# filthyrake/telescope_cam_detection

Hardware: AMD Instinct MI355X
Metric: frames_per_sec (higher is better)
Workload: dtype f16x3; 1 GPU; RT-DETR-R50 640x640 bs=8/GPU, uint8 BGR frames resident in HBM -> [8,300,6] detections in HBM; synthetic seeded weights; global_batch=8, parallelism=camera-shard x1, streams_per_gpu=1, batches_in_flight_per_gpu=1, hip_graph=True

## Files before the change

telescope_cam_detection_amd/_capi.py:

```python
from __future__ import annotations

import ctypes as C
import os
from typing import Optional

import numpy as np

from . import build as _build
from .arch import Arch

RTD_OK, RTD_E_INVALID, RTD_E_OOM, RTD_E_HIP, RTD_E_WEIGHTS, RTD_E_STATE = range(6)
PREC_BF16, PREC_FP32, PREC_F16X3 = 0, 1, 2
DT_BF16, DT_F32, DT_F16X2 = 0, 1, 4
SPLIT_GROUP = 32


def precision_code(name) -> int:
    if isinstance(name, int):
        return name
    s = str(name).lower()
    if s in ("f16x3", "fp16x3", "pair"):
        return PREC_F16X3
    if s in ("fp32", "f32", "float32"):
        return PREC_FP32
# ... 62 lines not shown

class RtdEnhanceParams(C.Structure):
    _fields_ = [("struct_size", C.c_int32), ("clip_limit", C.c_float), ("tiles_x", C.c_int32), ("tiles_y", C.c_int32),
                ("bilateral_d", C.c_int32), ("sigma_color", C.c_float), ("sigma_space", C.c_float)]


class RtdEsrganConfig(C.Structure):
    _fields_ = [("struct_size", C.c_int32), ("device", C.c_int32), ("precision", C.c_int32), ("num_feat", C.c_int32),
                ("num_grow_ch", C.c_int32), ("num_block", C.c_int32), ("tile", C.c_int32), ("tile_pad", C.c_int32)]


DET_DTYPE = np.dtype([("class_id", "<i4"), ("score", "<f4"), ("x1", "<f4"), ("y1", "<f4"), ("x2", "<f4"), ("y2", "<f4")])

_lib: Optional[C.CDLL] = None

EXPORTS = [
    "rtd_version", "rtd_create", "rtd_load_weights", "rtd_infer", "rtd_infer_raw", "rtd_infer_async", "rtd_collect", "rtd_prepare",
    "rtd_result_block", "rtd_sync", "rtd_stream", "rtd_wait_stream", "rtd_signal_stream", "rtd_get_stats", "rtd_arena_bytes", "rtd_destroy",
    "rtd_last_error", "rtd_crop_resize_batch", "rtd_self_check", "rtd_preprocess",
    "rtd_motion_create", "rtd_motion_check", "rtd_motion_reset", "rtd_motion_wait_stream", "rtd_motion_last_error", "rtd_motion_destroy",
    "rtd_mog2_create", "rtd_mog2_configure", "rtd_mog2_apply", "rtd_mog2_wait_stream", "rtd_mog2_last_error", "rtd_mog2_destroy",
    "rtd_jpeg_create", "rtd_jpeg_encode", "rtd_jpeg_wait_stream", "rtd_jpeg_last_error", "rtd_jpeg_destroy",
    "rtd_overlay_create", "rtd_overlay_draw", "rtd_overlay_wait_stream", "rtd_overlay_last_error", "rtd_overlay_destroy",
    "rtd_enhance_create", "rtd_enhance_layout", "rtd_enhance_crops", "rtd_enhance_last_error", "rtd_enhance_destroy",
    "rtd_esrgan_create", "rtd_esrgan_layout", "rtd_esrgan_upscale", "rtd_esrgan_arena_bytes", "rtd_esrgan_last_error", "rtd_esrgan_destroy",
]
TEST_EXPORTS = [
    "rtd_debug_tensor", "rtd_debug_force_topk", "rtd_profile", "rtd_debug_option", "rtd_op_conv", "rtd_op_conv_dual", "rtd_op_conv_next",
    "rtd_op_layernorm", "rtd_op_attention", "rtd_op_msdeform", "rtd_op_topk", "rtd_op_resize", "rtd_op_pool", "rtd_bench_conv", "rtd_bench_conv_pair",
    "rtd_bench_mfma_rate", "rtd_debug_motion_state", "rtd_debug_mog2_model", "rtd_debug_mog2_fg_bits",
    "rtd_debug_jpeg_coefficients", "rtd_debug_overlay_tiles", "rtd_debug_enhance_stage",
    "rtd_op_conv_view", "rtd_bench_conv_act", "rtd_debug_esrgan_tensor",
    "rtd_op_msdeform_view", "rtd_op_select_score", "rtd_op_gather_ln", "rtd_op_split_convert", "rtd_op_set_rows", "rtd_op_rowmax",
    "rtd_op_gather_rows", "rtd_op_boxes", "rtd_op_add", "rtd_op_postprocess",
]


def lib() -> C.CDLL:
    global _lib
    if _lib is not None:
        return _lib
    path = _build.LIB_PATH
    override = os.environ.get("RTD_LIB_PATH")
    if override:
        if not os.path.exists(override):
            raise RuntimeError(f"RTD_LIB_PATH={override} does not exist")
        path = override
    elif _build.needs_build():
        try:
            path = _build.build(verbose=False)
        except Exception as e:
            if not os.path.exists(path):
                raise RuntimeError(f"libmi355rtdetr.so is missing and cannot be built: {e}") from e
    try:
        import torch
    except Exception:
        pass
    L = C.CDLL(path)
    vp, i32, f32, i64 = C.c_void_p, C.c_int32, C.c_float, C.c_int64
    L.rtd_version.restype = C.c_char_p
    L.rtd_last_error.restype = C.c_char_p
    L.rtd_last_error.argtypes = [vp]
    L.rtd_create.argtypes = [C.POINTER(RtdConfig), C.POINTER(vp)]
    L.rtd_load_weights.argtypes = [vp, vp, C.c_size_t]
    L.rtd_infer.argtypes = [vp, i32, C.POINTER(vp), C.POINTER(i32), i32, f32, i32, vp, C.POINTER(i32)]
    L.rtd_infer_raw.argtypes = [vp, i32, C.POINTER(vp), C.POINTER(i32), i32, vp, vp, vp]
    L.rtd_infer_async.argtypes = [vp, i32, C.POINTER(vp), C.POINTER(i32), i32]
# ... 76 lines not shown
    if hasattr(L, "rtd_enhance_create"):
        L.rtd_enhance_create.argtypes = [i32, C.POINTER(RtdEnhanceParams), C.POINTER(vp)]
        L.rtd_enhance_layout.argtypes = [i32, C.POINTER(i32), C.POINTER(i64)]
        L.rtd_enhance_crops.argtypes = [vp, i32, C.POINTER(vp), C.POINTER(i32), C.POINTER(i32), vp, i64, vp]
        L.rtd_enhance_last_error.argtypes = [vp]
        L.rtd_enhance_last_error.restype = C.c_char_p
        L.rtd_enhance_destroy.argtypes = [vp]
        L.rtd_enhance_destroy.restype = None
        L.rtd_debug_enhance_stage.argtypes = [vp, i32, i32, vp, C.c_size_t]
    if hasattr(L, "rtd_esrgan_create"):
        L.rtd_esrgan_create.argtypes = [C.POINTER(RtdEsrganConfig), vp, C.c_size_t, C.POINTER(vp)]
        L.rtd_esrgan_layout.argtypes = [i32, C.POINTER(i32), C.POINTER(i64)]
        L.rtd_esrgan_upscale.argtypes = [vp, i32, C.POINTER(vp), C.POINTER(i32), C.POINTER(i32), vp, i64, vp]
        L.rtd_esrgan_arena_bytes.argtypes = [vp]
        L.rtd_esrgan_arena_bytes.restype = i64
        L.rtd_esrgan_last_error.argtypes = [vp]
        L.rtd_esrgan_last_error.restype = C.c_char_p
        L.rtd_esrgan_destroy.argtypes = [vp]
        L.rtd_esrgan_destroy.restype = None
        L.rtd_debug_esrgan_tensor.argtypes = [vp, C.c_char_p, vp, i64, C.POINTER(i64)]
        L.rtd_op_conv_view.argtypes = [i32, vp, i32, vp, vp, vp, i32, vp, i32] + [i32] * 10
        L.rtd_bench_conv_act.argtypes = [i32] * 13 + [C.POINTER(f32)]
    if hasattr(L, "rtd_op_select_score"):
        L.rtd_op_msdeform_view.argtypes = [i32, vp, i32, i32, vp, vp, vp] + [i32] * 6 + [C.POINTER(i32), f32]
        L.rtd_op_select_score.argtypes = [vp, i32, vp, vp, vp, vp, vp, i32, i32, i32, i32]
        L.rtd_op_gather_ln.argtypes = [vp, i32, i32, vp, i32, i32, vp, vp, vp, i32]
        L.rtd_op_split_convert.argtypes = [i32, vp, vp, i64, i32, i64, i64]
        L.rtd_op_set_rows.argtypes = [i32, vp, i32, i32, vp, i32, i32, vp, i32]
        L.rtd_op_rowmax.argtypes = [vp, i32, i32, i32, vp]
        L.rtd_op_gather_rows.argtypes = [i32, vp, i32, i32, vp, i32, i32, i32, vp, i32]
        L.rtd_op_boxes.argtypes = [vp, i32, i32, vp, vp, vp, i32, vp]
        L.rtd_op_add.argtypes = [i32, i32, i32, vp, vp, vp, i32, i32, i32, i32]
        L.rtd_op_postprocess.argtypes = [vp, vp, vp, i32, i32, i32, i32, i32, vp]
    _lib = L
    return L


def debug_option(name: str, value: int) -> None:
    rc = lib().rtd_debug_option(name.encode(), int(value))
    if rc != RTD_OK:
        raise ValueError(f"unknown debug option {name!r}")


class RtdError(RuntimeError):
    def __init__(self, code: int, msg: str):
        super().__init__(f"rtd error {code}: {msg}")
        self.code = code


def _stats_of(handle) -> dict:
    st = RtdStats()
    if not handle or lib().rtd_get_stats(handle, C.byref(st)) != RTD_OK:
        return {}
    return {k: (float(getattr(st, k)) if k == "max_abs_filter" else int(getattr(st, k))) for k, _ in RtdStats._fields_ if k not in ("struct_size", "reserved")}


def _raise_msg(code: int, what: str, msg: bytes, suffix: str = ""):
    msg = (msg or b"").decode(errors="replace") + suffix
    if code == RTD_E_OOM:
        import torch
        raise torch.cuda.OutOfMemoryError(f"HIP out of memory in {what}: {msg}")
    raise RtdError(code, msg)


def _raise(code: int, handle=None) -> None:
    assert handle is None
# ... 271 lines not shown
```

telescope_cam_detection_amd/csrc/common.h:

```cpp
#pragma once
#include <hip/hip_runtime.h>
#include <stdint.h>
#include <string.h>

#include <stdexcept>
#include <string>
#include <tuple>
#include <type_traits>
#include <utility>
#include <vector>

#include "error.h"

namespace rtd {

enum DType : int { BF16 = 0, F32 = 1, U8 = 2, I32 = 3, F16X2 = 4 };
constexpr int SPLIT_GROUP = 32;
enum Act : int { ACT_NONE = 0, ACT_RELU = 1, ACT_SILU = 2, ACT_GELU = 3, ACT_LRELU = 4  };
enum ResMode : int { RES_NONE = 0, RES_PRE = 1, RES_POST = 2 };

inline size_t dtype_size(int dt) { return dt == BF16 ? 2 : (dt == U8 ? 1 : 4); }

typedef __bf16 bf16;
typedef __bf16 bf16x8 __attribute__((ext_vector_type(8)));
// ... 138 lines not shown
                      float eps, hipStream_t s);
void launch_add(const Tensor& a, const Tensor& b, const Tensor& y, hipStream_t s);
void launch_axpby(float alpha, const Tensor& a, const Tensor& b, const Tensor& y, hipStream_t s);
void launch_maxpool3x3s2(const Tensor& x, const Tensor& y, hipStream_t s);
void launch_upsample2x(const Tensor& x, const Tensor& y, hipStream_t s);
void launch_avgpool2(const Tensor& x, const Tensor& y, hipStream_t s);
void launch_attention(const Tensor& qk, const Tensor& v, const Tensor& o, int heads, hipStream_t s);
void launch_set_rows(const Tensor& y, const int32_t* rows, int nrows, int rows_per_image, const float* vec,
                     hipStream_t s);
void launch_rowmax(const Tensor& x, float* out, hipStream_t s);
void launch_topk(const float* keys, int B, int N, int K, int32_t* idx, float* vals, hipStream_t s);
void launch_gather_rows(const Tensor& src, const int32_t* idx, int rows_per_image, const Tensor& dst, hipStream_t s);
void launch_ref_init(const Tensor& boxdelta, const float* anchors, const int32_t* idx, int S, float* ref_unact8,
                     float* ref8, hipStream_t s);
void launch_msdeform(const Tensor& value, int value_coff, const Tensor& offaw, const float* ref8, const Tensor& out,
                     int heads, int hd, int n_levels, int n_points, const int32_t* level_hw_start, float offset_scale,
                     hipStream_t s);
void launch_box_refine(const Tensor& delta, float* ref8, hipStream_t s);
void launch_postprocess_scores(const Tensor& logits, float* scores, hipStream_t s);
bool postprocess_fused_supported(const Tensor& logits, int B, int Q);
void launch_postprocess_fused(const Tensor& logits, const float* ref8, const float* scale_wh, int B, int Q, float* block6, hipStream_t s);
void launch_postprocess_gather(const float* topv, const int32_t* topi, const float* ref8, const float* scale_wh,
                               int B, int Q, int C, float* block6, hipStream_t s);
constexpr int RTD_MAX_BATCH = 64;
struct FrameArgs {
  const uint8_t* ptr[RTD_MAX_BATCH];
  float scale_wh[2 * RTD_MAX_BATCH];
  int n;
};
void launch_preprocess_identity(const FrameArgs& fa, int H, int W, const Tensor& y, float* scale_wh_dev, hipStream_t s);
void launch_set_scale(const FrameArgs& fa, float* scale_wh_dev, hipStream_t s);
void launch_set_frame_table(const FrameArgs& fa, const uint8_t** table_dev, float* scale_wh_dev, hipStream_t s);
void launch_stem0_u8(const uint8_t* const* table_dev, int n, int H, int W, const void* w, int Kpad, const float* bias, const Tensor& y, int act,
                     hipStream_t s);
struct ResizeCoef {
  const int32_t* hb;
  const int32_t* hk;
  const int32_t* vb;
  const int32_t* vk;
  int hks, vks;
};
void launch_resize_pil(const uint8_t* src, int sh, int sw, uint8_t* tmp, const Tensor& y, int image, const ResizeCoef& coef,
                       hipStream_t s);
void launch_u8_hwc_to_chw_f32(const uint8_t* src, int H, int W, float* out, hipStream_t s);
void launch_resize_pil_u8(const uint8_t* src, int sh, int sw, uint8_t* tmp, uint8_t* dst, int dh, int dw, const ResizeCoef& c, hipStream_t s);
struct DecLin {
  const float* w;
  const float* b;
  int ldw, N, K;
};
struct DecLN {
  const float* g;
  const float* b;
};

struct DecArgs {
  int mode;
  int attn_split;
  int split;
  int B, Q, D, heads, S, n_levels, n_points, ffn, C;
  float offset_scale;
  const float* q_in;
  const float* kfrag_in;
  const float* vfrag_in;
  const float* hs_in;
  float* hs_out;
  const float* qpos_in;
// ... 105 lines not shown
```

telescope_cam_detection_amd/csrc/engine.hip:

```cpp
#include "engine_internal.h"

using namespace rtd;
using namespace rtd_eng;

namespace rtd {
__thread GraphBuild* t_graph_build = nullptr;
__thread long long t_launches = 0;
}

void launch_force_idx(int32_t* dst, const int32_t* src, const int32_t* flag, int n, hipStream_t s);

namespace rtd_eng {
PlanOpts g_opts;
}

namespace rtd_eng {

void parse_blob(rtd_engine* e) {
  const char* b = e->blob.data();
  const size_t n = e->blob.size();
  RTD_CHECK(n >= 12 && memcmp(b, "RTDW", 4) == 0, RTD_E_WEIGHTS, "weight blob: bad magic");
  uint32_t ver, count;
  memcpy(&ver, b + 4, 4);
  memcpy(&count, b + 8, 4);
// ... 471 lines not shown
    int si, bi, stride, oh, ow, cin, cout;
    bool last, fold_sc;
    Tensor res, sc_in, out;
  };
  void stem(Flow& F);
  void backbone_stage(Flow& F, int si, int cin);
  void shortcut(Flow& F, Block& b);
  void bottleneck_body(Flow& F, const StageBufs& sb, const Block& b);
  void basic_body(Flow& F, const StageBufs& sb, const Block& b);
  Tensor aifi_fused(const Tensor& t0), aifi_by_op(const Tensor& t0);
  Tensor csp(const std::string& pfx, const Tensor& cat, const std::string& oname, const Tensor* up_src = nullptr);
  Tensor encoder(Flow& F);
  bool dec_fused() const { return e->opts.dec_fused && c.d_model == 256 && c.dec_heads == 8 && c.dec_ffn <= 1024 && c.num_classes <= 512 && c.n_levels == 3 && c.n_points == 4; }
  Queries select_queries(Flow& F, const Tensor& mem);
  Decoded decoder(Flow& F, const Tensor& mem, const Queries& q);
  Tensor decoder_fused(Flow& F, const Queries& q, const Tensor& vall, float* ref8, float* ref_unact8);
  Tensor decoder_by_op(const Queries& q, const Tensor& vall, const Tensor& ref8t, float* ref_unact8);
  void post_process(const Decoded& d);
};

void Builder::stem(Flow& F) {
  const int H = c.input_h, W = c.input_w;
  Tensor x = act(SP ? F32 : P, n, H, W, 8, "input");
  plan->input = x;
  const int eh = c.embedding_size / 2;
  const int h = down2(H), w = down2(W);
  Tensor s0 = act(P, n, h, w, eh);
  plan->stem_fused = SP && e->opts.stem_fused_split && eh == 32;
  if (plan->stem_fused) {
    const uint8_t** table = (const uint8_t**)alloc((size_t)c.max_batch * sizeof(void*));
    plan->frame_table = table;
    if (!dry) {
      DevWeight w0 = get_weight(e, {{"backbone.stem.0", 9 * 8}}, P, eh);
      const void* wp = w0.w; const float* bp = w0.bias; const int kp = w0.Kpad; const int n = this->n;
      push("backbone.stem.0", "conv_igemm", 2.0 * n * h * w * eh * 27.0, (double)n * H * W * 3 + tbytes(s0),
           [table, n, H, W, wp, kp, bp, s0](hipStream_t st) { launch_stem0_u8(table, n, H, W, wp, kp, bp, s0, ACT_RELU, st); });
    }
  } else {
    conv("backbone.stem.0", x, s0, {.k = 3, .stride = 2, .pad = 1, .act = ACT_RELU, .real_cin = 3});
  }
  Tensor s1 = act(P, n, h, w, eh);
  conv("backbone.stem.1", s0, s1, {.k = 3, .pad = 1, .act = ACT_RELU});
  const Tensor s2v = mk(nullptr, P, n, h, w, c.embedding_size);
  const int ph = down2(h), pw = down2(w);
  const ConvSpec stem2{.k = 3, .pad = 1, .act = ACT_RELU};
  const long long pool_tiles = (long long)n * ((w + 31) / 32) * ((h + 7) / 8);
  const bool fuse = SP && e->opts.stem_pool_fuse && conv_pool_supported(probe(s1, s2v, stem2), probe_shape(mk(nullptr, P, n, ph, pw, c.embedding_size), 1)) &&
                    pool_tiles * 8192 < (1ll << 31);
  F.h = ph; F.w = pw;
  if (fuse) {
    F.cur = act(P, n, ph, pw, c.embedding_size, "stem");
    ConvArgs a;
    a.x = s1; a.y = s2v;
    a.KH = a.KW = 3; a.stride = 1; a.pad = 1; a.act = ACT_RELU; a.opts = &e->conv_opts;
    const DevWeight w2 = get_weight(e, {{"backbone.stem.2", 9 * s1.c}}, P, c.embedding_size, dry);
    a.w = w2.w; a.bias = w2.bias; a.Kpad = w2.Kpad; a.Npad = w2.Npad;
    void* side = alloc(conv_pool_side_bytes(a));
    const Tensor curv = F.cur;
    push("backbone.stem.2+pool", "conv_igemm", 2.0 * s2v.pixels() * s2v.c * 9.0 * s1.c, tbytes(s1) + tbytes(curv),
         [a, curv, side](hipStream_t st) { launch_conv_pool(a, curv, side, st); });
  } else {
    Tensor s2 = act(P, n, h, w, c.embedding_size);
    conv("backbone.stem.2", s1, s2, stem2);
    F.cur = act(P, n, ph, pw, c.embedding_size, "stem");
    const Tensor curv = F.cur;
    push("backbone.pool", "maxpool", 9.0 * curv.pixels() * curv.c, tbytes(s2) + tbytes(curv),
         [s2, curv](hipStream_t s) { launch_maxpool3x3s2(s2, curv, s); });
  }
}
// ... 1064 lines not shown
```

telescope_cam_detection_amd/csrc/engine_internal.h:

```cpp
#pragma once
#include <math.h>
#include <string.h>

#include <chrono>
#include <functional>
#include <map>
#include <memory>
#include <mutex>
#include <string>
#include <vector>

#include "../../include/rtdetr_mi355_test.h"
#include "backend.h"

namespace rtd_eng {
using namespace rtd;

struct PlanOpts {
  int sc_fold = 1;
  int c1_fuse = 1;
  int attn_split = 3;
  int up_fold = 1;
  int arena_reuse = 1;
  int stem_fused_split = 1;
  int aifi_pair = 1;
  int post_fused = 1;
  int dead_out = 1;
  int avg_fuse = 1;
  int stem_pool_fuse = 1;
  int sel_fused = 1;
  int dec_fused = 1;
  int side_stream = 7;
};

struct HostTensor {
  const float* data = nullptr;
  std::vector<int64_t> shape;
  int64_t numel() const {
    int64_t n = 1;
    for (auto d : shape) n *= d;
    return n;
  }
};

struct DevWeight {
  void* w = nullptr;
  float* bias = nullptr;
  int N = 0, K = 0, Kpad = 0, Npad = 0, dt = F32;
};

struct Op {
  std::string name;
  const char* kernel;
  double flops, bytes;
  std::function<void(hipStream_t)> run;
  bool debug_only = false;
  int lane = 0, kind = 0;
// ... 106 lines not shown
```

telescope_cam_detection_amd/csrc/ops.hip:

```cpp
#include <float.h>

#include <algorithm>

#include "common.h"

namespace rtd {

template <typename T> __device__ __forceinline__ float ldf(const T* p) { return (float)(*p); }
template <typename T> __device__ __forceinline__ void stf(T* p, float v) { *p = (T)v; }

__device__ __forceinline__ float wave_sum(float v) { return wave_sum64(v); }

static inline unsigned blocks_for(int64_t n, int per_block) { return (unsigned)((n + per_block - 1) / per_block); }

template <typename... KArgs, typename... Args>
static void launch_1d(void (*kernel)(KArgs...), int64_t total, hipStream_t s, Args&&... args) {
  rtd_launch(kernel, dim3(blocks_for(total, 256)), dim3(256), 0, s, std::forward<Args>(args)...);
  HIP_CHECK(hipGetLastError());
}

template <typename T> struct TypeTag { typedef T type; };
template <typename Tag> using type_of = typename Tag::type;
template <typename F>
static void with_dtype(int dt, F&& f) {
// ... 1084 lines not shown
    o[2] = (T)((float)v[0] / 255.0f);
#pragma unroll
    for (int q = 3; q < 8; ++q) o[q] = (T)0.f;
  }
}
void launch_resize_pil(const uint8_t* src, int sh, int sw, uint8_t* tmp, const Tensor& y, int image, const ResizeCoef& c,
                       hipStream_t s) {
  const int dh = y.h, dw = y.w;
  RTD_CHECK(y.c == 8 && y.ld == 8 && image < y.n, 1, "resize: output must be [n,H,W,8]");
  launch_1d(k_resize_h, (int64_t)sh * dw, s, src, sh, sw, tmp, dw, c);
  char* yp = (char*)y.p + (size_t)image * y.bstride * dtype_size(y.dt);
  with_dtype(y.dt, [&](auto t) { typedef type_of<decltype(t)> T; launch_1d(k_resize_v<T>, (int64_t)dh * dw, s, tmp, sh, dw, (T*)yp, dh, c); });
}
void launch_resize_pil_u8(const uint8_t* src, int sh, int sw, uint8_t* tmp, uint8_t* dst, int dh, int dw, const ResizeCoef& c, hipStream_t s) {
  launch_1d(k_resize_h, (int64_t)sh * dw, s, src, sh, sw, tmp, dw, c);
  launch_1d(k_resize_v<uint8_t>, (int64_t)dh * dw, s, tmp, sh, dw, dst, dh, c);
}

__global__ void k_u8_hwc_to_chw_f32(const uint8_t* __restrict__ src, int H, int W, float* __restrict__ out) {
  const int64_t i = (int64_t)blockIdx.x * blockDim.x + threadIdx.x;
  const int64_t hw = (int64_t)H * W;
  if (i >= hw) return;
  const uint8_t* px = src + i * 3;
  out[i] = (float)px[2] / 255.0f;
  out[hw + i] = (float)px[1] / 255.0f;
  out[2 * hw + i] = (float)px[0] / 255.0f;
}
void launch_u8_hwc_to_chw_f32(const uint8_t* src, int H, int W, float* out, hipStream_t s) {
  launch_1d(k_u8_hwc_to_chw_f32, (int64_t)H * W, s, src, H, W, out);
}

typedef float f32x16_s __attribute__((ext_vector_type(16)));
typedef float f32x4_s __attribute__((ext_vector_type(4)));
__global__ __launch_bounds__(256) void stem0_u8_kernel(const uint8_t* const* __restrict__ table, int H, int W, const sp16* __restrict__ wq, int Kpad,
                                                        const float* __restrict__ bias, sp16* __restrict__ y, long long y_bstride, long long ldy,
                                                        int OH, int OW, int tiles_x, int tiles_y, int act) {
  constexpr bool SPLIT = true;
  typedef sp16 E;
  typedef E Ex8 __attribute__((ext_vector_type(8)));
  typedef E Ex4 __attribute__((ext_vector_type(4)));
  constexpr int TH = 8, TW = 32, PR = 2 * TH + 1, PC = 2 * TW + 1, ROWE = 200;
  constexpr int NDW = (PC * 3 + 3 + 3) / 4;
  constexpr int ROWO = (SPLIT ? 128 : 64) + 16;
  __shared__ __attribute__((aligned(16))) E patch[PR * ROWE];
  __shared__ __attribute__((aligned(16))) E patch_lo[SPLIT ? PR * ROWE : 8];
  __shared__ __attribute__((aligned(16))) char stage[4][32 * ROWO];
  const int tid = threadIdx.x, lane = tid & 63, wv = tid >> 6, h = lane >> 5;
  int t = blockIdx.x;
  const int tx = t % tiles_x; t /= tiles_x;
  const int ty = t % tiles_y;
  const int b = t / tiles_y;
  const int x0 = tx * TW, y0 = ty * TH;
  const uint8_t* __restrict__ f = table[b];
  const long long fbytes = (long long)H * W * 3;
  const bool aligned4 = (((uintptr_t)f) & 3) == 0;
  for (int e = tid; e < PR * NDW; e += 256) {
    const int r = e / NDW, d = e - r * NDW;
    const int iy = 2 * y0 - 1 + r;
    const long long g0 = ((long long)iy * W + (2 * x0 - 1)) * 3;
    const long long a0 = (g0 & ~3ll) + 4ll * d;
    unsigned dw = 0;
    const bool row_ok = (unsigned)iy < (unsigned)H;
    if (row_ok) {
      if (aligned4 && a0 >= 0 && a0 + 4 <= fbytes) dw = *(const unsigned*)(f + a0);
      else {
#pragma unroll
        for (int q = 0; q < 4; ++q)
          if (a0 + q >= 0 && a0 + q < fbytes) dw |= (unsigned)f[a0 + q] << (8 * q);
      }
    }
#pragma unroll
    for (int q = 0; q < 4; ++q) {
      const int el = (int)(a0 + q - g0);
      if (el < 0 || el >= PC * 3) continue;
      const int ix = 2 * x0 - 1 + el / 3;
      const float v = (row_ok && (unsigned)ix < (unsigned)W) ? (float)((dw >> (8 * q)) & 0xffu) : 0.f;
      const float vn = v / 255.0f;
      const E hi = (E)vn;
      patch[r * ROWE + el] = hi;
      if (SPLIT) patch_lo[r * ROWE + el] = (E)(vn - (float)hi);
    }
  }
  for (int e = tid; e < PR * (ROWE - PC * 3); e += 256) {
    const int r = e / (ROWE - PC * 3), i = e - r * (ROWE - PC * 3);
    patch[r * ROWE + PC * 3 + i] = (E)0.f;
    if (SPLIT) patch_lo[r * ROWE + PC * 3 + i] = (E)0.f;
  }
  Ex8 wf[2], wfl[2];
  int doff[2][4];
#pragma unroll
  for (int s = 0; s < 2; ++s) {
#pragma unroll
    for (int j = 0; j < 8; ++j) {
      const int k = 16 * s + 8 * h + j;
      const int kh = k / 10, e = k - kh * 10;
      const int kw = e / 3, cb = e - kw * 3;
      const int kr = (kh * 3 + kw) * 8 + (2 - cb);
      const bool real = k < 30 && e < 9;
      if (SPLIT) {
        const size_t pos = (size_t)(lane & 31) * Kpad + ((kr >> 5) << 6) + (kr & 31);
        wf[s][j] = real ? wq[pos] : (E)0.f;
        wfl[s][j] = real ? wq[pos + 32] : (E)0.f;
      } else {
        wf[s][j] = real ? wq[(size_t)(lane & 31) * Kpad + kr] : (E)0.f;
      }
    }
#pragma unroll
    for (int j = 0; j < 4; ++j) {
      const int k = 16 * s + 8 * h + 2 * j;
      const int kh = k / 10, e = k - kh * 10;
      doff[s][j] = k < 30 ? kh * ROWE + e : 0;
    }
  }
  __syncthreads();
#pragma unroll 1
  for (int rr = 0; rr < 2; ++rr) {
    const int r = wv * 2 + rr;
    const int eoff = (2 * r) * ROWE + (2 * (lane & 31)) * 3;
    const E* base = patch + eoff;
    f32x16_s acc;
#pragma unroll
    for (int e = 0; e < 16; ++e) acc[e] = 0.f;
#pragma unroll
    for (int s = 0; s < 2; ++s) {
      typedef unsigned u4_s __attribute__((ext_vector_type(4)));
      unsigned xd[4];
#pragma unroll
      for (int j = 0; j < 4; ++j) xd[j] = *(const unsigned*)(base + doff[s][j]);
      const u4_s xv = {xd[0], xd[1], xd[2], xd[3]};
      if constexpr (SPLIT) acc = mfma_pair32(wf[s], __builtin_bit_cast(Ex8, xv), acc);
      else acc = __builtin_amdgcn_mfma_f32_32x32x16_bf16(wf[s], __builtin_bit_cast(Ex8, xv), acc, 0, 0, 0);
      if constexpr (SPLIT) {
        unsigned xl[4];
#pragma unroll
        for (int j = 0; j < 4; ++j) xl[j] = *(const unsigned*)(patch_lo + eoff + doff[s][j]);
        const u4_s xlv = {xl[0], xl[1], xl[2], xl[3]};
        acc = mfma_pair32(wf[s], __builtin_bit_cast(Ex8, xlv), acc);
        acc = mfma_pair32(wfl[s], __builtin_bit_cast(Ex8, xv), acc);
      }
    }
    const int oy = y0 + r;
    char* sw_ = stage[wv];
#pragma unroll
    for (int q = 0; q < 4; ++q) {
      const f32x4_s bv = *(const f32x4_s*)(bias + 8 * q + 4 * h);
      Ex4 o, ol;
#pragma unroll
      for (int e = 0; e < 4; ++e) {
        float v = acc[4 * q + e] + bv[e];
        if (act == ACT_RELU) v = fmaxf(v, 0.f);
        else if (act == ACT_SILU) v = v / (1.f + __expf(-v));
        if constexpr (SPLIT) { sp16 hh, ll; split2(v, hh, ll); o[e] = hh; ol[e] = ll; }
        else o[e] = (E)v;
      }
      *(Ex4*)(sw_ + (lane & 31) * ROWO + (8 * q + 4 * h) * 2) = o;
      if (SPLIT) *(Ex4*)(sw_ + (lane & 31) * ROWO + 64 + (8 * q + 4 * h) * 2) = ol;
    }
    __builtin_amdgcn_wave_barrier();
    if (oy < OH) {
      constexpr int CPP = SPLIT ? 8 : 4;
      E* yrow = y + (SPLIT ? 2 : 1) * ((long long)b * y_bstride + ((long long)oy * OW + x0) * ldy);
#pragma unroll
      for (int i2 = 0; i2 < CPP / 2; ++i2) {
        const int idx = i2 * 64 + lane;
        const int p = idx / CPP, ch = idx % CPP;
        if (x0 + p < OW) *(Ex8*)(yrow + (SPLIT ? 2 : 1) * (long long)p * ldy + ch * 8) = *(const Ex8*)(sw_ + p * ROWO + ch * 16);
      }
    }
    __builtin_amdgcn_wave_barrier();
  }
}
void launch_stem0_u8(const uint8_t* const* table_dev, int n, int H, int W, const void* w, int Kpad, const float* bias, const Tensor& y, int act,
                     hipStream_t s) {
  const int OH = (H + 2 - 3) / 2 + 1, OW = (W + 2 - 3) / 2 + 1;
  RTD_CHECK(y.dt == F16X2 && y.c == 32 && y.h == OH && y.w == OW && y.n >= n && y.ld % SPLIT_GROUP == 0 &&
                (act == ACT_RELU || act == ACT_NONE || act == ACT_SILU), 1, "stem0_u8: output must be F16X2 [n, H/2, W/2, 32]");
  const int tiles_x = (OW + 31) / 32, tiles_y = (OH + 7) / 8;
  rtd_launch(stem0_u8_kernel, dim3((unsigned)(n * tiles_x * tiles_y)), dim3(256), 0, s, table_dev, H, W, (const sp16*)w, Kpad, bias, (sp16*)y.p,
                     (long long)y.bstride, (long long)y.ld, OH, OW, tiles_x, tiles_y, act);
  HIP_CHECK(hipGetLastError());
}

struct CropNorm { float mean[3], inv_std[3]; };
__global__ void k_crop_resize(const CropBatch cb, int n, int S, CropNorm nm, float* __restrict__ out) {
  const int64_t i = (int64_t)blockIdx.x * blockDim.x + threadIdx.x;
  const int64_t per = (int64_t)S * S;
  if (i >= per * n) return;
  const int c = (int)(i / per);
  const int p = (int)(i - (int64_t)c * per);
  const int oy = p / S, ox = p - oy * S;
  const int cw = cb.x2[c] - cb.x1[c], chh = cb.y2[c] - cb.y1[c];
  const float sx = (float)cw / (float)S, sy = (float)chh / (float)S;
  const float fx = fmaxf(sx * ((float)ox + 0.5f) - 0.5f, 0.f), fy = fmaxf(sy * ((float)oy + 0.5f) - 0.5f, 0.f);
  const int x0 = min((int)fx, cw - 1), y0 = min((int)fy, chh - 1);
  const int x1 = min(x0 + 1, cw - 1), y1 = min(y0 + 1, chh - 1);
  const float lx1 = fx - (float)x0, ly1 = fy - (float)y0, lx0 = 1.f - lx1, ly0 = 1.f - ly1;
  const uint8_t* f = cb.frame[c];
  const int64_t fw = cb.fw[c];
  const uint8_t* p00 = f + ((int64_t)(cb.y1[c] + y0) * fw + cb.x1[c] + x0) * 3;
  const uint8_t* p01 = f + ((int64_t)(cb.y1[c] + y0) * fw + cb.x1[c] + x1) * 3;
  const uint8_t* p10 = f + ((int64_t)(cb.y1[c] + y1) * fw + cb.x1[c] + x0) * 3;
  const uint8_t* p11 = f + ((int64_t)(cb.y1[c] + y1) * fw + cb.x1[c] + x1) * 3;
#pragma unroll
  for (int ch = 0; ch < 3; ++ch) {
    const int sc = 2 - ch;
    const float v = ly0 * (lx0 * (float)p00[sc] + lx1 * (float)p01[sc]) + ly1 * (lx0 * (float)p10[sc] + lx1 * (float)p11[sc]);
    out[((int64_t)c * 3 + ch) * per + p] = (v / 255.0f - nm.mean[ch]) * nm.inv_std[ch];
  }
}
void launch_crop_resize(const CropBatch& cb, int n, int out_size, const float mean[3], const float stdv[3], float* out, hipStream_t s) {
  RTD_CHECK(n >= 1 && n <= 64 && out_size >= 1 && out_size <= 4096, 1, "crop batch: 1..64 crops per launch");
  for (int i = 0; i < n; ++i) {
// ... 11 lines not shown
```

telescope_cam_detection_amd/csrc/testapi.hip:

```cpp
#include "engine_internal.h"

using namespace rtd;
using namespace rtd_eng;

struct OpScratch {
  std::vector<void*> bufs;
  template <typename T> T* get(size_t count) {
    void* p = nullptr;
    HIP_CHECK(hipMalloc(&p, count ? count * sizeof(T) : 16));
    bufs.push_back(p);
    return (T*)p;
  }
  template <typename T> T* upload(const T* host, size_t count) {
    T* d = get<T>(count);
    HIP_CHECK(hipMemcpy(d, host, count * sizeof(T), hipMemcpyHostToDevice));
    return d;
  }
  ~OpScratch() { for (void* p : bufs) (void)hipFree(p); }
};
static bool rows_fit_int(int a, int b) { return a >= 1 && b >= 1 && (int64_t)a * b <= 0x7fffffff; }
static Tensor rows_view(const void* p, int dt, int n, int rows, int c, int64_t ld) {
  Tensor t = mk(p, dt, n, rows, 1, c);
  t.ld = ld; t.bstride = (int64_t)rows * ld;
  return t;
// ... 151 lines not shown
  sp16x8 a[4], b[4];
  for (int i = 0; i < 4; ++i)
    for (int j = 0; j < 8; ++j) {
      const unsigned h = seed[(lane * 8 + j + i * 512) & 4095];
      a[i][j] = __builtin_bit_cast(sp16, (unsigned short)h);
      b[i][j] = __builtin_bit_cast(sp16, (unsigned short)(h >> 16));
    }
  f32x4 acc[16];
  for (int i = 0; i < 16; ++i) acc[i] = f32x4{0.f, 0.f, 0.f, 0.f};
  const long long c0 = __builtin_amdgcn_s_memtime(), r0 = __builtin_amdgcn_s_memrealtime();
  for (int it = 0; it < iters; ++it) {
#pragma unroll
    for (int i = 0; i < 16; ++i) asm volatile("v_mfma_f32_16x16x32_f16 %0, %1, %2, %0" : "+v"(acc[i]) : "v"(a[i & 3]), "v"(b[(i >> 2) & 3]));
  }
  asm volatile("s_nop 15\n\ts_nop 15\n\ts_nop 15" ::: "memory");
  __builtin_amdgcn_s_waitcnt(0);
  const long long c1 = __builtin_amdgcn_s_memtime(), r1 = __builtin_amdgcn_s_memrealtime();
  float s = 0.f;
  for (int i = 0; i < 16; ++i) s += acc[i][0] + acc[i][3];
  if (s == 123.456f) sink[0] = s;
  if (lane == 0) { const int w = blockIdx.x * 4 + (tid >> 6); out[2 * w] = c1 - c0; out[2 * w + 1] = r1 - r0; }
}
static int g_bench_rewarm = 0;
int rtd_debug_option(const char* name, int value) {
  if (!name) return RTD_E_INVALID;
  if (strcmp(name, "reset") == 0) {
    g_opts = PlanOpts();
    g_profile_twice = 0; g_bench_rewarm = 0;
    conv_opts_template() = ConvOpts();
    return RTD_OK;
  }
  const struct { const char* n; int* p; } plan_opts[] = {
      {"dec_fused", &g_opts.dec_fused}, {"side_stream", &g_opts.side_stream}, {"sel_fused", &g_opts.sel_fused},
      {"stem_fused_split", &g_opts.stem_fused_split}, {"stem_pool_fuse", &g_opts.stem_pool_fuse}, {"avg_fuse", &g_opts.avg_fuse}, {"dead_out", &g_opts.dead_out}, {"post_fused", &g_opts.post_fused}, {"aifi_pair", &g_opts.aifi_pair}, {"sc_fold", &g_opts.sc_fold}, {"arena_reuse", &g_opts.arena_reuse},
      {"up_fold", &g_opts.up_fold}, {"attn_split", &g_opts.attn_split}, {"c1_fuse", &g_opts.c1_fuse},
      {"profile_twice", &g_profile_twice}, {"bench_rewarm", &g_bench_rewarm},
  };
  for (const auto& t : plan_opts)
    if (strcmp(name, t.n) == 0) { *t.p = value; return RTD_OK; }
  if (conv_set_option(name, value)) return RTD_OK;
  return RTD_E_INVALID;
}

struct DevFilter {
  float* wpad = nullptr; void* w = nullptr; float* bias = nullptr;
  int Kpad = 0, Npad = 0;
  void release() { if (w != wpad) (void)hipFree(w); (void)hipFree(wpad); (void)hipFree(bias); }
};
static DevFilter dev_filter(int dtype, const void* w_f32, const float* bias, int N, int K) {
  DevFilter f;
  f.Npad = conv_npad(N);
  f.Kpad = dtype == F16X2 ? conv_kpad_split(K) : conv_kpad(K);
  const int kcols = dtype == F16X2 ? f.Kpad / 2 : f.Kpad;
  HIP_CHECK(hipMalloc((void**)&f.wpad, (size_t)f.Npad * kcols * 4));
  HIP_CHECK(hipMemset(f.wpad, 0, (size_t)f.Npad * kcols * 4));
  HIP_CHECK(hipMemcpy2D(f.wpad, (size_t)kcols * 4, w_f32, (size_t)K * 4, (size_t)K * 4, N, hipMemcpyDeviceToDevice));
  HIP_CHECK(hipMalloc((void**)&f.bias, (size_t)f.Npad * 4));
  HIP_CHECK(hipMemset(f.bias, 0, (size_t)f.Npad * 4));
  HIP_CHECK(hipMemcpy(f.bias, bias, (size_t)N * 4, hipMemcpyDeviceToDevice));
  f.w = f.wpad;
  if (dtype == BF16 || dtype == F16X2) HIP_CHECK(hipMalloc(&f.w, (size_t)f.Npad * f.Kpad * 2));
  if (dtype == BF16) launch_f32_to(f.wpad, f.w, BF16, (int64_t)f.Npad * f.Kpad, nullptr);
  else if (dtype == F16X2) launch_f32_to_split(f.wpad, kcols, f.w, kcols, f.Npad, kcols, nullptr);
  return f;
}

static int op_conv_impl(int dtype, const void* x, const void* x2, int C2, const void* w_ohwi_f32, const float* bias, const void* res, void* y,
// ... 218 lines not shown
    const int cus = prop.multiProcessorCount;
    std::vector<unsigned> hs(4096, 0u);
    if (random_operands)
      for (int i = 0; i < 4096; ++i) {
        unsigned h = (unsigned)i * 2654435761u + 12345u; h ^= h >> 15; h *= 2246822519u; h ^= h >> 13;
        const unsigned lo = (h & 0x8000u) | ((10u + ((h >> 20) & 7u)) << 10) | (h & 0x3ffu);
        unsigned h2 = h * 2654435761u; h2 ^= h2 >> 16;
        const unsigned hi = (h2 & 0x8000u) | ((10u + ((h2 >> 20) & 7u)) << 10) | (h2 & 0x3ffu);
        hs[i] = lo | (hi << 16);
      }
    Scratch sc;
    HIP_CHECK(hipMalloc((void**)&sc.seed, 4096 * 4)); HIP_CHECK(hipMalloc((void**)&sc.stamps, (size_t)cus * 4 * 2 * 8)); HIP_CHECK(hipMalloc((void**)&sc.sink, 16));
    HIP_CHECK(hipMemcpy(sc.seed, hs.data(), 4096 * 4, hipMemcpyHostToDevice));
    const int iters = ms_target * 9400;
    HIP_CHECK(hipEventCreate(&sc.e0)); HIP_CHECK(hipEventCreate(&sc.e1));
    float ms = 0.f;
    for (int rep = 0; rep < 3; ++rep) {
      HIP_CHECK(hipEventRecord(sc.e0, nullptr));
      rtd_launch(k_mfma_rate, dim3(cus), dim3(256), 0, nullptr, sc.seed, iters, sc.stamps, sc.sink);
      HIP_CHECK(hipEventRecord(sc.e1, nullptr));
      HIP_CHECK(hipEventSynchronize(sc.e1));
      HIP_CHECK(hipEventElapsedTime(&ms, sc.e0, sc.e1));
    }
    std::vector<long long> h((size_t)cus * 4 * 2);
    HIP_CHECK(hipMemcpy(h.data(), sc.stamps, h.size() * 8, hipMemcpyDeviceToHost));
    double cyc = 0, rt = 0;
    for (int w = 0; w < cus * 4; ++w) { cyc += (double)h[2 * w]; rt += (double)h[2 * w + 1]; }
    out[0] = (float)((double)iters * 16.0 * cus * 4.0 * 16384.0 / (ms * 1e-3) / 1e12);
    out[1] = (float)(cyc / (rt * 10.0));
    out[2] = ms;
  });
}

int rtd_op_layernorm(int dtype, const void* x, const void* res, const float* g, const float* b, void* y, int rows, int dim, int out_f32) {
  return op_guard([&] {
    Tensor tx = mk(x, dtype, 1, rows, 1, dim), ty = mk(y, out_f32 ? F32 : dtype, 1, rows, 1, dim), tr = mk(res, dtype, 1, rows, 1, dim);
    launch_layernorm(tx, res ? &tr : nullptr, g, b, ty, 1e-5f, nullptr);
  });
}

int rtd_op_attention(int dtype, const void* qk, const void* v, void* o, int B, int L, int heads, int hd) {
  return op_guard([&] {
    const int D = heads * hd;
    launch_attention(mk(qk, dtype, B, L, 1, 2 * D), mk(v, dtype, B, L, 1, D), mk(o, dtype, B, L, 1, D), heads, nullptr);
  });
}

int rtd_op_msdeform(int dtype, const void* value, const float* offaw, const float* ref, float* out, int B, int Q, int heads, int hd,
                    int n_levels, int n_points, const int32_t* level_hw, int value_ld, float offset_scale) {
  return op_guard([&] {
    RTD_CHECK(n_levels >= 1 && n_levels <= 8, RTD_E_INVALID, "n_levels");
    int32_t lv[24]; int S = 0;
    for (int l = 0; l < n_levels; ++l) { lv[l * 3] = level_hw[2 * l]; lv[l * 3 + 1] = level_hw[2 * l + 1]; lv[l * 3 + 2] = S; S += level_hw[2 * l] * level_hw[2 * l + 1]; }
    int32_t* lvd = nullptr; float* ref8 = nullptr;
    HIP_CHECK(hipMalloc((void**)&lvd, sizeof lv));
    HIP_CHECK(hipMemcpy(lvd, lv, sizeof lv, hipMemcpyHostToDevice));
    HIP_CHECK(hipMalloc((void**)&ref8, (size_t)B * Q * 32));
    HIP_CHECK(hipMemset(ref8, 0, (size_t)B * Q * 32));
    HIP_CHECK(hipMemcpy2D(ref8, 32, ref, 16, 16, (size_t)B * Q, hipMemcpyDeviceToDevice));
    Tensor tv = mk(value, dtype, B, S, 1, heads * hd);
    tv.ld = value_ld; tv.bstride = (int64_t)S * value_ld;
    launch_msdeform(tv, 0, mk(offaw, F32, B, Q, 1, heads * n_levels * n_points * 3), ref8, mk(out, F32, B, Q, 1, heads * hd), heads, hd,
                    n_levels, n_points, lvd, offset_scale, nullptr);
    HIP_CHECK(hipDeviceSynchronize());
    (void)hipFree(lvd); (void)hipFree(ref8);
  });
// ... 169 lines not shown
```

Before: 1849 frames/s.

## Make stem0 u8 conv kernel persistent with double-buffered patch prefetch

Turns the first stem convolution, which reads uint8 frames directly, into a persistent kernel with a grid capped at 768 blocks. Each block loops over tiles and prefetches the next tile's raw bytes into registers while the current tile runs its MFMAs, with the converted patch double-buffered in LDS. It also swaps the per-element divide-and-split for a 256-entry LUT, makes the activation a template parameter, hoists the bias loads, and writes output through buffer stores with out-of-range masking. The cost is more LDS and register pressure, which may lower occupancy, plus extra per-tile bookkeeping.

Result: no change. 1855 frames/s (median of 6 runs) (+0.3%).

```diff
diff --git a/telescope_cam_detection_amd/_capi.py b/telescope_cam_detection_amd/_capi.py
--- a/telescope_cam_detection_amd/_capi.py
+++ b/telescope_cam_detection_amd/_capi.py
@@ -118,7 +118,7 @@
     "rtd_debug_jpeg_coefficients", "rtd_debug_overlay_tiles", "rtd_debug_enhance_stage",
     "rtd_op_conv_view", "rtd_bench_conv_act", "rtd_debug_esrgan_tensor",
     "rtd_op_msdeform_view", "rtd_op_select_score", "rtd_op_gather_ln", "rtd_op_split_convert", "rtd_op_set_rows", "rtd_op_rowmax",
-    "rtd_op_gather_rows", "rtd_op_boxes", "rtd_op_add", "rtd_op_postprocess",
+    "rtd_op_gather_rows", "rtd_op_boxes", "rtd_op_add", "rtd_op_postprocess", "rtd_op_stem0_u8",
 ]
 
 
@@ -261,6 +261,8 @@
         L.rtd_op_boxes.argtypes = [vp, i32, i32, vp, vp, vp, i32, vp]
         L.rtd_op_add.argtypes = [i32, i32, i32, vp, vp, vp, i32, i32, i32, i32]
         L.rtd_op_postprocess.argtypes = [vp, vp, vp, i32, i32, i32, i32, i32, vp]
+    if hasattr(L, "rtd_op_stem0_u8"):
+        L.rtd_op_stem0_u8.argtypes = [C.POINTER(vp), i32, i32, i32, vp, vp, vp, i32]
     _lib = L
     return L
 
diff --git a/telescope_cam_detection_amd/csrc/common.h b/telescope_cam_detection_amd/csrc/common.h
--- a/telescope_cam_detection_amd/csrc/common.h
+++ b/telescope_cam_detection_amd/csrc/common.h
@@ -194,7 +194,7 @@
 void launch_set_scale(const FrameArgs& fa, float* scale_wh_dev, hipStream_t s);
 void launch_set_frame_table(const FrameArgs& fa, const uint8_t** table_dev, float* scale_wh_dev, hipStream_t s);
 void launch_stem0_u8(const uint8_t* const* table_dev, int n, int H, int W, const void* w, int Kpad, const float* bias, const Tensor& y, int act,
-                     hipStream_t s);
+                     int persist, hipStream_t s);
 struct ResizeCoef {
   const int32_t* hb;
   const int32_t* hk;
diff --git a/telescope_cam_detection_amd/csrc/engine.hip b/telescope_cam_detection_amd/csrc/engine.hip
--- a/telescope_cam_detection_amd/csrc/engine.hip
+++ b/telescope_cam_detection_amd/csrc/engine.hip
@@ -527,9 +527,9 @@
     plan->frame_table = table;
     if (!dry) {
       DevWeight w0 = get_weight(e, {{"backbone.stem.0", 9 * 8}}, P, eh);
-      const void* wp = w0.w; const float* bp = w0.bias; const int kp = w0.Kpad; const int n = this->n;
+      const void* wp = w0.w; const float* bp = w0.bias; const int kp = w0.Kpad; const int n = this->n; const int persist = e->opts.stem0_persist;
       push("backbone.stem.0", "conv_igemm", 2.0 * n * h * w * eh * 27.0, (double)n * H * W * 3 + tbytes(s0),
-           [table, n, H, W, wp, kp, bp, s0](hipStream_t st) { launch_stem0_u8(table, n, H, W, wp, kp, bp, s0, ACT_RELU, st); });
+           [table, n, H, W, wp, kp, bp, s0, persist](hipStream_t st) { launch_stem0_u8(table, n, H, W, wp, kp, bp, s0, ACT_RELU, persist, st); });
     }
   } else {
     conv("backbone.stem.0", x, s0, {.k = 3, .stride = 2, .pad = 1, .act = ACT_RELU, .real_cin = 3});
diff --git a/telescope_cam_detection_amd/csrc/engine_internal.h b/telescope_cam_detection_amd/csrc/engine_internal.h
--- a/telescope_cam_detection_amd/csrc/engine_internal.h
+++ b/telescope_cam_detection_amd/csrc/engine_internal.h
@@ -23,6 +23,7 @@
   int up_fold = 1;
   int arena_reuse = 1;
   int stem_fused_split = 1;
+  int stem0_persist = 768;
   int aifi_pair = 1;
   int post_fused = 1;
   int dead_out = 1;
diff --git a/telescope_cam_detection_amd/csrc/ops.hip b/telescope_cam_detection_amd/csrc/ops.hip
--- a/telescope_cam_detection_amd/csrc/ops.hip
+++ b/telescope_cam_detection_amd/csrc/ops.hip
@@ -1140,59 +1140,86 @@
 
 typedef float f32x16_s __attribute__((ext_vector_type(16)));
 typedef float f32x4_s __attribute__((ext_vector_type(4)));
+template <bool PERSIST, int ACT>
 __global__ __launch_bounds__(256) void stem0_u8_kernel(const uint8_t* const* __restrict__ table, int H, int W, const sp16* __restrict__ wq, int Kpad,
                                                         const float* __restrict__ bias, sp16* __restrict__ y, long long y_bstride, long long ldy,
-                                                        int OH, int OW, int tiles_x, int tiles_y, int act) {
+                                                        int OH, int OW, int tiles_x, int tiles_y, int ntiles, unsigned y_bytes) {
   constexpr bool SPLIT = true;
   typedef sp16 E;
   typedef E Ex8 __attribute__((ext_vector_type(8)));
   typedef E Ex4 __attribute__((ext_vector_type(4)));
   constexpr int TH = 8, TW = 32, PR = 2 * TH + 1, PC = 2 * TW + 1, ROWE = 200;
   constexpr int NDW = (PC * 3 + 3 + 3) / 4;
+  constexpr int NLD = (PR * NDW + 255) / 256;
   constexpr int ROWO = (SPLIT ? 128 : 64) + 16;
-  __shared__ __attribute__((aligned(16))) E patch[PR * ROWE];
-  __shared__ __attribute__((aligned(16))) E patch_lo[SPLIT ? PR * ROWE : 8];
+  constexpr int NBUF = PERSIST ? 2 : 1;
+  constexpr int PSZ = PR * ROWE + 8;
+  __shared__ __attribute__((aligned(16))) E patch[NBUF][PSZ];
+  __shared__ __attribute__((aligned(16))) E patch_lo[NBUF][SPLIT ? PSZ : 8];
+  __shared__ unsigned lut[256];
   __shared__ __attribute__((aligned(16))) char stage[4][32 * ROWO];
   const int tid = threadIdx.x, lane = tid & 63, wv = tid >> 6, h = lane >> 5;
   int t = blockIdx.x;
-  const int tx = t % tiles_x; t /= tiles_x;
-  const int ty = t % tiles_y;
-  const int b = t / tiles_y;
-  const int x0 = tx * TW, y0 = ty * TH;
-  const uint8_t* __restrict__ f = table[b];
+  int tx = t % tiles_x, ty = (t / tiles_x) % tiles_y, b = t / (tiles_x * tiles_y);
+  const int G = (int)gridDim.x, gtx = G % tiles_x, gty = (G / tiles_x) % tiles_y, gb = G / (tiles_x * tiles_y);
   const long long fbytes = (long long)H * W * 3;
-  const bool aligned4 = (((uintptr_t)f) & 3) == 0;
-  for (int e = tid; e < PR * NDW; e += 256) {
-    const int r = e / NDW, d = e - r * NDW;
-    const int iy = 2 * y0 - 1 + r;
-    const long long g0 = ((long long)iy * W + (2 * x0 - 1)) * 3;
-    const long long a0 = (g0 & ~3ll) + 4ll * d;
-    unsigned dw = 0;
-    const bool row_ok = (unsigned)iy < (unsigned)H;
-    if (row_ok) {
-      if (aligned4 && a0 >= 0 && a0 + 4 <= fbytes) dw = *(const unsigned*)(f + a0);
-      else {
-#pragma unroll
-        for (int q = 0; q < 4; ++q)
-          if (a0 + q >= 0 && a0 + q < fbytes) dw |= (unsigned)f[a0 + q] << (8 * q);
-      }
-    }
-#pragma unroll
-    for (int q = 0; q < 4; ++q) {
-      const int el = (int)(a0 + q - g0);
-      if (el < 0 || el >= PC * 3) continue;
-      const int ix = 2 * x0 - 1 + el / 3;
-      const float v = (row_ok && (unsigned)ix < (unsigned)W) ? (float)((dw >> (8 * q)) & 0xffu) : 0.f;
-      const float vn = v / 255.0f;
-      const E hi = (E)vn;
-      patch[r * ROWE + el] = hi;
-      if (SPLIT) patch_lo[r * ROWE + el] = (E)(vn - (float)hi);
-    }
-  }
-  for (int e = tid; e < PR * (ROWE - PC * 3); e += 256) {
+  auto load_patch = [&](int b_, int y0, int x0, unsigned (&dw)[NLD]) {
+    const uint8_t* __restrict__ f = table[b_];
+    const bool aligned4 = (((uintptr_t)f) & 3) == 0;
+#pragma unroll
+    for (int i = 0; i < NLD; ++i) {
+      const int e = tid + 256 * i, r = e / NDW, d = e - r * NDW;
+      const int iy = 2 * y0 - 1 + r;
+      const long long g0 = ((long long)iy * W + (2 * x0 - 1)) * 3;
+      const long long a0 = (g0 & ~3ll) + 4ll * d;
+      dw[i] = 0;
+      if (e < PR * NDW && (unsigned)iy < (unsigned)H) {
+        if (aligned4 && a0 >= 0 && a0 + 4 <= fbytes) dw[i] = *(const unsigned*)(f + a0);
+        else {
+#pragma unroll
+          for (int q = 0; q < 4; ++q)
+            if (a0 + q >= 0 && a0 + q < fbytes) dw[i] |= (unsigned)f[a0 + q] << (8 * q);
+        }
+      }
+    }
+  };
+  auto convert_patch = [&](int buf, int y0, int x0, const unsigned (&dw)[NLD]) {
+#pragma unroll
+    for (int i = 0; i < NLD; ++i) {
+      const int e = tid + 256 * i, r = e / NDW, d = e - r * NDW;
+      if (e >= PR * NDW) continue;
+      const int iy = 2 * y0 - 1 + r;
+      const long long g0 = ((long long)iy * W + (2 * x0 - 1)) * 3;
+      const int el0 = 4 * d - (int)(g0 & 3);
+      const bool row_ok = (unsigned)iy < (unsigned)H;
+#pragma unroll
+      for (int q = 0; q < 4; ++q) {
+        const int el = el0 + q;
+        const bool in_row = el >= 0 && el < PC * 3;
+        const int ix = 2 * x0 - 1 + el / 3;
+        const unsigned v = (row_ok && in_row && (unsigned)ix < (unsigned)W) ? ((dw[i] >> (8 * q)) & 0xffu) : 0u;
+        const unsigned pr = lut[v];
+        const int at = in_row ? r * ROWE + el : PR * ROWE;
+        patch[buf][at] = __builtin_bit_cast(E, (unsigned short)pr);
+        if (SPLIT) patch_lo[buf][at] = __builtin_bit_cast(E, (unsigned short)(pr >> 16));
+      }
+    }
+  };
+  unsigned dw[NLD];
+  load_patch(b, ty * TH, tx * TW, dw);
+  {
+    const float vn = (float)tid / 255.0f;
+    const E hi = (E)vn, lo = (E)(vn - (float)hi);
+    lut[tid] = (unsigned)__builtin_bit_cast(unsigned short, hi) | (unsigned)__builtin_bit_cast(unsigned short, lo) << 16;
+  }
+  f32x4_s bv[4];
+#pragma unroll
+  for (int q = 0; q < 4; ++q) bv[q] = *(const f32x4_s*)(bias + 8 * q + 4 * h);
+  for (int e = tid; e < NBUF * PR * (ROWE - PC * 3); e += 256) {
     const int r = e / (ROWE - PC * 3), i = e - r * (ROWE - PC * 3);
-    patch[r * ROWE + PC * 3 + i] = (E)0.f;
-    if (SPLIT) patch_lo[r * ROWE + PC * 3 + i] = (E)0.f;
+    const int at = (r / PR) * PSZ + (r % PR) * ROWE + PC * 3 + i;
+    (&patch[0][0])[at] = (E)0.f;
+    if (SPLIT) (&patch_lo[0][0])[at] = (E)0.f;
   }
   Ex8 wf[2], wfl[2];
   int doff[2][4];
@@ -1221,71 +1248,98 @@
     }
   }
   __syncthreads();
-#pragma unroll 1
-  for (int rr = 0; rr < 2; ++rr) {
-    const int r = wv * 2 + rr;
-    const int eoff = (2 * r) * ROWE + (2 * (lane & 31)) * 3;
-    const E* base = patch + eoff;
-    f32x16_s acc;
-#pragma unroll
-    for (int e = 0; e < 16; ++e) acc[e] = 0.f;
-#pragma unroll
-    for (int s = 0; s < 2; ++s) {
-      typedef unsigned u4_s __attribute__((ext_vector_type(4)));
-      unsigned xd[4];
-#pragma unroll
-      for (int j = 0; j < 4; ++j) xd[j] = *(const unsigned*)(base + doff[s][j]);
-      const u4_s xv = {xd[0], xd[1], xd[2], xd[3]};
-      if constexpr (SPLIT) acc = mfma_pair32(wf[s], __builtin_bit_cast(Ex8, xv), acc);
-      else acc = __builtin_amdgcn_mfma_f32_32x32x16_bf16(wf[s], __builtin_bit_cast(Ex8, xv), acc, 0, 0, 0);
-      if constexpr (SPLIT) {
-        unsigned xl[4];
-#pragma unroll
-        for (int j = 0; j < 4; ++j) xl[j] = *(const unsigned*)(patch_lo + eoff + doff[s][j]);
-        const u4_s xlv = {xl[0], xl[1], xl[2], xl[3]};
-        acc = mfma_pair32(wf[s], __builtin_bit_cast(Ex8, xlv), acc);
-        acc = mfma_pair32(wfl[s], __builtin_bit_cast(Ex8, xv), acc);
-      }
-    }
-    const int oy = y0 + r;
-    char* sw_ = stage[wv];
-#pragma unroll
-    for (int q = 0; q < 4; ++q) {
-      const f32x4_s bv = *(const f32x4_s*)(bias + 8 * q + 4 * h);
-      Ex4 o, ol;
-#pragma unroll
-      for (int e = 0; e < 4; ++e) {
-        float v = acc[4 * q + e] + bv[e];
-        if (act == ACT_RELU) v = fmaxf(v, 0.f);
-        else if (act == ACT_SILU) v = v / (1.f + __expf(-v));
-        if constexpr (SPLIT) { sp16 hh, ll; split2(v, hh, ll); o[e] = hh; ol[e] = ll; }
-        else o[e] = (E)v;
-      }
-      *(Ex4*)(sw_ + (lane & 31) * ROWO + (8 * q + 4 * h) * 2) = o;
-      if (SPLIT) *(Ex4*)(sw_ + (lane & 31) * ROWO + 64 + (8 * q + 4 * h) * 2) = ol;
-    }
-    __builtin_amdgcn_wave_barrier();
-    if (oy < OH) {
-      constexpr int CPP = SPLIT ? 8 : 4;
-      E* yrow = y + (SPLIT ? 2 : 1) * ((long long)b * y_bstride + ((long long)oy * OW + x0) * ldy);
-#pragma unroll
-      for (int i2 = 0; i2 < CPP / 2; ++i2) {
-        const int idx = i2 * 64 + lane;
-        const int p = idx / CPP, ch = idx % CPP;
-        if (x0 + p < OW) *(Ex8*)(yrow + (SPLIT ? 2 : 1) * (long long)p * ldy + ch * 8) = *(const Ex8*)(sw_ + p * ROWO + ch * 16);
-      }
-    }
-    __builtin_amdgcn_wave_barrier();
+  convert_patch(0, ty * TH, tx * TW, dw);
+  for (int cur = 0;; cur ^= NBUF - 1) {
+    __syncthreads();
+    const int x0 = tx * TW, y0 = ty * TH;
+    int nt = t + G, ntx = tx + gtx, nty = ty + gty, nb = b + gb;
+    if (ntx >= tiles_x) { ntx -= tiles_x; ++nty; }
+    if (nty >= tiles_y) { nty -= tiles_y; ++nb; }
+    const bool more = PERSIST && nt < ntiles;
+    if (more) load_patch(nb, nty * TH, ntx * TW, dw);
+    const __amdgpu_buffer_rsrc_t ry = __builtin_amdgcn_make_buffer_rsrc((void*)(y + (SPLIT ? 2 : 1) * (long long)b * y_bstride), 0, y_bytes, 0x00020000);
+#pragma unroll
+    for (int rr = 0; rr < 2; ++rr) {
+      const int r = wv * 2 + rr;
+      const int eoff = (2 * r) * ROWE + (2 * (lane & 31)) * 3;
+      const E* base = patch[cur] + eoff;
+      f32x16_s acc;
+#pragma unroll
+      for (int e = 0; e < 16; ++e) acc[e] = 0.f;
+#pragma unroll
+      for (int s = 0; s < 2; ++s) {
+        typedef unsigned u4_s __attribute__((ext_vector_type(4)));
+        unsigned xd[4];
+#pragma unroll
+        for (int j = 0; j < 4; ++j) xd[j] = *(const unsigned*)(base + doff[s][j]);
+        const u4_s xv = {xd[0], xd[1], xd[2], xd[3]};
+        if constexpr (SPLIT) acc = mfma_pair32(wf[s], __builtin_bit_cast(Ex8, xv), acc);
+        else acc = __builtin_amdgcn_mfma_f32_32x32x16_bf16(wf[s], __builtin_bit_cast(Ex8, xv), acc, 0, 0, 0);
+        if constexpr (SPLIT) {
+          unsigned xl[4];
+#pragma unroll
+          for (int j = 0; j < 4; ++j) xl[j] = *(const unsigned*)(patch_lo[cur] + eoff + doff[s][j]);
+          const u4_s xlv = {xl[0], xl[1], xl[2], xl[3]};
+          acc = mfma_pair32(wf[s], __builtin_bit_cast(Ex8, xlv), acc);
+          acc = mfma_pair32(wfl[s], __builtin_bit_cast(Ex8, xv), acc);
+        }
+      }
+      const int oy = y0 + r;
+      char* sw_ = stage[wv];
+#pragma unroll
+      for (int q = 0; q < 4; ++q) {
+        Ex4 o, ol;
+#pragma unroll
+        for (int e = 0; e < 4; ++e) {
+          float v = acc[4 * q + e] + bv[q][e];
+          if (ACT == ACT_RELU) v = fmaxf(v, 0.f);
+          else if (ACT == ACT_SILU) v = v / (1.f + __expf(-v));
+          if constexpr (SPLIT) { sp16 hh, ll; split2(v, hh, ll); o[e] = hh; ol[e] = ll; }
+          else o[e] = (E)v;
+        }
+        *(Ex4*)(sw_ + (lane & 31) * ROWO + (8 * q + 4 * h) * 2) = o;
+        if (SPLIT) *(Ex4*)(sw_ + (lane & 31) * ROWO + 64 + (8 * q + 4 * h) * 2) = ol;
+      }
+      __builtin_amdgcn_wave_barrier();
+      {
+        constexpr int CPP = SPLIT ? 8 : 4;
+        typedef unsigned u4_o __attribute__((ext_vector_type(4)));
+#pragma unroll
+        for (int i2 = 0; i2 < CPP / 2; ++i2) {
+          const int idx = i2 * 64 + lane;
+          const int p = idx / CPP, ch = idx % CPP;
+          const unsigned off = (oy < OH && x0 + p < OW) ? (unsigned)((SPLIT ? 4 : 2) * ((long long)oy * OW + x0 + p) * ldy + ch * 16) : 0x80000000u;
+          __builtin_amdgcn_raw_buffer_store_b128(*(const u4_o*)(sw_ + p * ROWO + ch * 16), ry, off, 0, 0);
+        }
+      }
+      __builtin_amdgcn_wave_barrier();
+    }
+    if (!more) break;
+    convert_patch(cur ^ 1, nty * TH, ntx * TW, dw);
+    t = nt; tx = ntx; ty = nty; b = nb;
   }
 }
 void launch_stem0_u8(const uint8_t* const* table_dev, int n, int H, int W, const void* w, int Kpad, const float* bias, const Tensor& y, int act,
-                     hipStream_t s) {
+                     int persist, hipStream_t s) {
   const int OH = (H + 2 - 3) / 2 + 1, OW = (W + 2 - 3) / 2 + 1;
   RTD_CHECK(y.dt == F16X2 && y.c == 32 && y.h == OH && y.w == OW && y.n >= n && y.ld % SPLIT_GROUP == 0 &&
-                (act == ACT_RELU || act == ACT_NONE || act == ACT_SILU), 1, "stem0_u8: output must be F16X2 [n, H/2, W/2, 32]");
+                (act == ACT_RELU || act == ACT_NONE || act == ACT_SILU) && persist >= 0, 1, "stem0_u8: output must be F16X2 [n, H/2, W/2, 32]");
   const int tiles_x = (OW + 31) / 32, tiles_y = (OH + 7) / 8;
-  rtd_launch(stem0_u8_kernel, dim3((unsigned)(n * tiles_x * tiles_y)), dim3(256), 0, s, table_dev, H, W, (const sp16*)w, Kpad, bias, (sp16*)y.p,
-                     (long long)y.bstride, (long long)y.ld, OH, OW, tiles_x, tiles_y, act);
+  const long long ntiles = (long long)n * tiles_x * tiles_y;
+  const long long y_bytes = 4 * (((long long)OH * OW - 1) * y.ld + 32);
+  RTD_CHECK(n >= 1 && ntiles <= 0x7fffffff && y_bytes < (1ll << 31), 1, "stem0_u8: tile count / image extent");
+  const long long grid = persist ? std::min<long long>(ntiles, persist) : ntiles;
+  auto go = [&](auto kernel) {
+    rtd_launch(kernel, dim3((unsigned)grid), dim3(256), 0, s, table_dev, H, W, (const sp16*)w, Kpad, bias, (sp16*)y.p, (long long)y.bstride,
+               (long long)y.ld, OH, OW, tiles_x, tiles_y, (int)ntiles, (unsigned)y_bytes);
+  };
+  auto with_act = [&](auto pc) {
+    constexpr bool P = decltype(pc)::value;
+    if (act == ACT_RELU) go(stem0_u8_kernel<P, ACT_RELU>);
+    else if (act == ACT_SILU) go(stem0_u8_kernel<P, ACT_SILU>);
+    else go(stem0_u8_kernel<P, ACT_NONE>);
+  };
+  if (persist) with_act(std::true_type{}); else with_act(std::false_type{});
   HIP_CHECK(hipGetLastError());
 }
 
diff --git a/telescope_cam_detection_amd/csrc/testapi.hip b/telescope_cam_detection_amd/csrc/testapi.hip
--- a/telescope_cam_detection_amd/csrc/testapi.hip
+++ b/telescope_cam_detection_amd/csrc/testapi.hip
@@ -207,7 +207,7 @@
   }
   const struct { const char* n; int* p; } plan_opts[] = {
       {"dec_fused", &g_opts.dec_fused}, {"side_stream", &g_opts.side_stream}, {"sel_fused", &g_opts.sel_fused},
-      {"stem_fused_split", &g_opts.stem_fused_split}, {"stem_pool_fuse", &g_opts.stem_pool_fuse}, {"avg_fuse", &g_opts.avg_fuse}, {"dead_out", &g_opts.dead_out}, {"post_fused", &g_opts.post_fused}, {"aifi_pair", &g_opts.aifi_pair}, {"sc_fold", &g_opts.sc_fold}, {"arena_reuse", &g_opts.arena_reuse},
+      {"stem_fused_split", &g_opts.stem_fused_split}, {"stem0_persist", &g_opts.stem0_persist}, {"stem_pool_fuse", &g_opts.stem_pool_fuse}, {"avg_fuse", &g_opts.avg_fuse}, {"dead_out", &g_opts.dead_out}, {"post_fused", &g_opts.post_fused}, {"aifi_pair", &g_opts.aifi_pair}, {"sc_fold", &g_opts.sc_fold}, {"arena_reuse", &g_opts.arena_reuse},
       {"up_fold", &g_opts.up_fold}, {"attn_split", &g_opts.attn_split}, {"c1_fuse", &g_opts.c1_fuse},
       {"profile_twice", &g_profile_twice}, {"bench_rewarm", &g_bench_rewarm},
   };
@@ -492,6 +492,20 @@
   });
 }
 
+int rtd_op_stem0_u8(const uint8_t* const* frames, int n, int H, int W, const float* w_ohwi_f32, const float* bias, void* y, int act) {
+  return op_guard([&] {
+    RTD_CHECK(frames && w_ohwi_f32 && bias && y && n >= 1 && H >= 1 && W >= 1, RTD_E_INVALID, "stem0_u8: arguments");
+    for (int i = 0; i < n; ++i) RTD_CHECK(frames[i], RTD_E_INVALID, "stem0_u8: frame pointer");
+    RTD_CHECK(g_opts.stem0_persist >= 0, RTD_E_INVALID, "stem0_persist: a grid size, or 0");
+    DevFilter f = dev_filter(F16X2, w_ohwi_f32, bias, 32, 9 * 8);
+    OpScratch sc;
+    const uint8_t* const* table = sc.upload(frames, (size_t)n);
+    launch_stem0_u8(table, n, H, W, f.w, f.Kpad, f.bias, mk(y, F16X2, n, (H - 1) / 2 + 1, (W - 1) / 2 + 1, 32), act, g_opts.stem0_persist, nullptr);
+    HIP_CHECK(hipDeviceSynchronize());
+    f.release();
+  });
+}
+
 int rtd_op_layernorm(int dtype, const void* x, const void* res, const float* g, const float* b, void* y, int rows, int dim, int out_f32) {
   return op_guard([&] {
     Tensor tx = mk(x, dtype, 1, rows, 1, dim), ty = mk(y, out_f32 ? F32 : dtype, 1, rows, 1, dim), tr = mk(res, dtype, 1, rows, 1, dim);
```
